# andimarafioti/faster-qwen3-tts

Hardware: NVIDIA H100
Metric: xRealTime (RTF) Qwen3-TTS-1.7B streaming chunk_size=8 (p50 TTFA in config) (higher is better)
Workload: dtype bf16

## Files before the change

### faster-qwen3-tts_b200/csrc/fq3_decode.cuh

```cuda
#pragma once
#include <cuda_bf16.h>
#include <cuda_runtime.h>
#include <stdint.h>

#include <type_traits>

#include "../../include/fq3_engine.h"

namespace fq3 {

constexpr int NCW = 8;
constexpr int NCT = NCW * 32;
constexpr int NTHREADS = NCT + 32;
constexpr int NS = 5;
constexpr int STAGE_BYTES = 32768;
constexpr int XS_FLOATS = 6144;
constexpr int HMAX = 2048;
constexpr int VMAX = 4096;
constexpr int MAXGRP = 512;
constexpr int MAXSEG = 256;
constexpr int SEQMAX = 4096;

enum Mode { MODE_FUSED = 0, MODE_TALKER_STEP = 1, MODE_PRED_RUN = 2, MODE_GEMV_TEST = 3 };

// ... 13 lines not shown
  float temperature, top_p, penalty;
};

struct StackDev {
  int H, I, L, nH, nKV, V, qd, kd, rep;
  float eps;
  int seg_base;
  int seg_head;
  const void *ln_in, *ln_post, *qnorm, *knorm, *ln_f;
  int S;
  const float *cos, *sin;
  int npos;
};

constexpr int KV_PAGE = 64;
__host__ __device__ __forceinline__ size_t kv_half_bytes(int L, int nKV, size_t esz) {
  return (size_t)L * nKV * KV_PAGE * 128 * esz;
}
__host__ __device__ __forceinline__ uint8_t* kv_row(void* pool, int L, int nKV, size_t esz, const int* pages, int which,
                                                    int layer, int g, int t) {
  const int page = pages[t / KV_PAGE];
  const size_t half = kv_half_bytes(L, nKV, esz);
  return reinterpret_cast<uint8_t*>(pool) + (size_t)page * 2 * half + (size_t)which * half +
         ((size_t)(layer * nKV + g) * KV_PAGE + t % KV_PAGE) * 128 * esz;
}

enum StateWord { ST_TOKEN = 0, ST_STEP = 1, ST_GEN = 2, ST_FIN = 3, ST_EMIT = 4, ST_WORDS = 5 };

struct SlotParams {
  void* kv;
  const int* kv_pages;
  void *pkc, *pvc;
  int* state;
  float* past_hidden;
  uint32_t* seen;
  const void* trailing;
  const void* tts_pad;
  const float* uniforms;
  long long* codes_out;
  float* logprob_out;
  int prefill_len, rope_delta, n_left_pad, max_new, min_new, trailing_len;
  int text_open;
  int n_frames;
  Sampling sp_t, sp_p;
};

struct KParams {
  StackDev t, p;
  int mode, ncta, nseg, seg_mtp;
  const uint8_t* tape;
  const Grp* grps;
  const uint32_t* segtab;
  const uint32_t* cta_grp_off;
  float *X, *X1, *QKV, *ACT, *LOGITS;
  void* ATT;
  int ldX, ldQKV, ldATT, ldACT;
  unsigned* bar;
  const void* t_embed;
  const void* p_embeds;
  const void* mtp_b;
  const void* mtp_tab;
  int has_mtp, ncb, eos, max_seq_len;
  SlotParams req;
  int n_frames;
  const void* in_embeds;
  void* hidden_out;
  int position;
  const void* pred_input;
  const float* pred_uniforms;
  float* dbg;
  int dbg_on;
  long long dbg_stride_layer;
  int attn_split;
  float* PART;
  unsigned* attn_cnt;
  int nslots;
  const SlotParams* sl;
  float *XB, *X1B, *QKVB, *LOGB;
  void *XNB, *ATTB, *ACTB, *PINB;
  int* TOKB;
  int gt_seg, gt_K, gt_ncols, gt_rows, gt_swiglu;
  const void* gt_x;
  void* gt_out;
};

__device__ __forceinline__ uint32_t smem_u32(const void* p) { return (uint32_t)__cvta_generic_to_shared(p); }
__device__ __forceinline__ void mbar_init(uint64_t* b, uint32_t cnt) {
  asm volatile("mbarrier.init.shared::cta.b64 [%0], %1;" ::"r"(smem_u32(b)), "r"(cnt) : "memory");
}
__device__ __forceinline__ void mbar_expect_tx(uint64_t* b, uint32_t bytes) {
  asm volatile("mbarrier.arrive.expect_tx.shared::cta.b64 _, [%0], %1;" ::"r"(smem_u32(b)), "r"(bytes) : "memory");
}
__device__ __forceinline__ void mbar_arrive(uint64_t* b) {
  asm volatile("mbarrier.arrive.shared::cta.b64 _, [%0];" ::"r"(smem_u32(b)) : "memory");
}
__device__ __forceinline__ bool mbar_try_wait(uint64_t* b, uint32_t parity) {
  uint32_t ok;
  asm volatile(
      "{\n\t.reg .pred p;\n\t"
      "mbarrier.try_wait.parity.shared::cta.b64 p, [%1], %2;\n\t"
      "selp.u32 %0, 1, 0, p;\n\t}"
      : "=r"(ok)
      : "r"(smem_u32(b)), "r"(parity)
      : "memory");
  return ok != 0;
}
__device__ __forceinline__ void mbar_wait(uint64_t* b, uint32_t parity) {
  while (!mbar_try_wait(b, parity)) {
// ... 812 lines not shown
    SMEM().ibc[3] = -1;
    SMEM().ibc[0] = 0x7fffffff;
  }
  csync();
  float woff = 0.f, total = 0.f;
  for (int w = 0; w < NCW; ++w) {
    if (w == c.warp) woff = total;
    total += SMEM().red[w];
  }
  incl += woff;
  const float target = a.u * total;
  float excl = __shfl_up_sync(0xffffffffu, incl, 1);
  if (c.lane == 0) excl = woff;
  const bool hit = incl > target;
  if (hit) atomicMin(&SMEM().ibc[0], c.tid);
  csync();
  if (hit && SMEM().ibc[0] == c.tid) {
    float run = excl;
    int pick = -1;
    for (int j = 0; j < CH; ++j) {
      const int idx = c.tid * CH + j;
      if (idx >= V) break;
      run += lg[idx];
      if (run > target && lg[idx] > 0.f) { pick = idx; break; }
    }
    SMEM().ibc[3] = pick;
  }
  csync();
  int tok = SMEM().ibc[3];
  if (tok < 0) {
    int best = -1;
    for (int v = c.tid; v < V; v += NCT)
      if (lg[v] > 0.f) best = v > best ? v : best;
#pragma unroll
    for (int o = 16; o; o >>= 1) best = max(best, __shfl_xor_sync(0xffffffffu, best, o));
    if (c.lane == 0) SMEM().hist[c.warp] = best;
    csync();
    tok = SMEM().hist[0];
    for (int w = 1; w < NCW; ++w) tok = max(tok, SMEM().hist[w]);
    if (tok < 0) tok = 0;
  }
  if (a.lp && c.tid == 0) *a.lp = (lraw[tok] - mx) - logf(sm);
  csync();
  return tok;
}

__device__ __forceinline__ void mma_bf16(float* d, const uint4& a, uint32_t b0, uint32_t b1) {
  asm volatile(
      "mma.sync.aligned.m16n8k16.row.col.f32.bf16.bf16.f32 {%0,%1,%2,%3}, {%4,%5,%6,%7}, {%8,%9}, {%0,%1,%2,%3};"
      : "+f"(d[0]), "+f"(d[1]), "+f"(d[2]), "+f"(d[3])
      : "r"(a.x), "r"(a.y), "r"(a.z), "r"(a.w), "r"(b0), "r"(b1));
}

template <int NT, class Pre, class Epi>
__device__ __forceinline__ void gemv_mma(Ctx& c, int seg, int K, Pre pre, Epi epi) {
  const __nv_bfloat16* xh = reinterpret_cast<const __nv_bfloat16*>(SMEM().xs);
  float* red = SMEM().xs + XS_FLOATS / 2;
  const uint32_t st = SMEM().seg[seg];
  const int gbeg = (int)(st >> 8), gn = (int)(st & 255u);
  const int gq = c.lane >> 2, t = c.lane & 3;
  for (int gi = 0; gi < gn; ++gi) {
    const Grp g = SMEM().grp[gbeg + gi];
    const int n_mt = g.rows & 0xff, kind = g.rows >> 8, G = g.m;
    int tok, koff;
    bool bvalid;
    if (kind == 1) { tok = gq >> 1; koff = (gq & 1) * (K >> 1); bvalid = gq < 2 * NT; }
    else { tok = gq; koff = 0; bvalid = gq < NT; }
    const __nv_bfloat16* xb = xh + (bvalid ? tok * K + koff : 0) + 16 * t;
    float aux[4] = {0.f, 0.f, 0.f, 0.f};
    if (c.warp < n_mt) {
      if (kind == 0) {
        const int rA = g.row0 + c.warp * 16 + gq;
        if (2 * t < NT) { aux[0] = pre(rA, 2 * t); aux[2] = pre(rA + 8, 2 * t); }
        if (2 * t + 1 < NT) { aux[1] = pre(rA, 2 * t + 1); aux[3] = pre(rA + 8, 2 * t + 1); }
      } else if (kind == 1) {
        if (t < NT) aux[0] = pre(g.row0 + gq, t);
      }
    }
    float acc[2][4];
#pragma unroll
    for (int a = 0; a < 2; ++a)
#pragma unroll
      for (int r = 0; r < 4; ++r) acc[a][r] = 0.f;
    for (int tl = 0; tl < g.ntiles; ++tl) {
      const int stage = (int)(c.tile_ctr % NS);
      const uint32_t par = (c.tile_ctr / NS) & 1u;
      mbar_wait(&SMEM().full[stage], par);
      const uint8_t* tile = SMEM().ring[stage];
      for (int qq = c.warp; qq < G; qq += NCW) {
        const int kg = tl * G + qq;
        uint4 blo = make_uint4(0, 0, 0, 0), bhi = make_uint4(0, 0, 0, 0);
        if (bvalid) {
          blo = *reinterpret_cast<const uint4*>(xb + 64 * kg);
          bhi = *reinterpret_cast<const uint4*>(xb + 64 * kg + 8);
        }
#pragma unroll
        for (int mt = 0; mt < 2; ++mt) {
          if (mt < n_mt) {
            const uint4* A = reinterpret_cast<const uint4*>(tile + ((size_t)(mt * G + qq) * 4) * 512) + c.lane;
            const uint4 a0 = A[0], a1 = A[32], a2 = A[64], a3 = A[96];
            mma_bf16(acc[mt], a0, blo.x, blo.y);
            mma_bf16(acc[mt], a1, blo.z, blo.w);
            mma_bf16(acc[mt], a2, bhi.x, bhi.y);
            mma_bf16(acc[mt], a3, bhi.z, bhi.w);
          }
        }
      }
      __syncwarp();
      if (c.lane == 0) mbar_arrive(&SMEM().empty[stage]);
      c.tile_ctr++;
    }
#pragma unroll
    for (int mt = 0; mt < 2; ++mt)
      if (mt < n_mt)
#pragma unroll
        for (int r = 0; r < 4; ++r) red[((c.warp * 2 + mt) * 4 + r) * 32 + c.lane] = acc[mt][r];
    csync();
    if (c.warp < n_mt) {
      const int mt = c.warp;
      float cv[4];
#pragma unroll
      for (int r = 0; r < 4; ++r) {
        float sm = 0.f;
#pragma unroll
        for (int w = 0; w < NCW; ++w) sm += red[((w * 2 + mt) * 4 + r) * 32 + c.lane];
        cv[r] = sm;
      }
      if (kind == 2) {
        const int pair = g.row0 + mt * 8 + gq;
        if (2 * t < NT) epi(pair, 2 * t, cv[0], cv[2], 0.f);
        if (2 * t + 1 < NT) epi(pair, 2 * t + 1, cv[1], cv[3], 0.f);
      } else if (kind == 0) {
        const int rA = g.row0 + mt * 16 + gq;
        if (2 * t < NT) { epi(rA, 2 * t, cv[0], 0.f, aux[0]); epi(rA + 8, 2 * t, cv[2], 0.f, aux[2]); }
        if (2 * t + 1 < NT) { epi(rA, 2 * t + 1, cv[1], 0.f, aux[1]); epi(rA + 8, 2 * t + 1, cv[3], 0.f, aux[3]); }
      } else {
        if (t < NT) epi(g.row0 + gq, t, cv[0] + cv[3], 0.f, aux[0]);
      }
    }
    csync();
  }
}

template <bool BF, bool GU, class Pre, class Epi>
__device__ __forceinline__ void gemv_any(Ctx& c, int seg, int nt, int K, Pre pre, Epi epi) {
  if constexpr (BF) {
    if (nt == 1) gemv_mma<1>(c, seg, K, pre, epi);
    else gemv_mma<2>(c, seg, K, pre, epi);
  } else {
    auto epi2 = [&](int row0, const float* v0, const float* v1) {
      for (int t = 0; t < nt; ++t) {
        if constexpr (GU) {
          epi(row0 >> 1, t, v0[t], v1[t], 0.f);
        } else {
          epi(row0, t, v0[t], 0.f, pre(row0, t));
          epi(row0 + 1, t, v1[t], 0.f, pre(row0 + 1, t));
        }
      }
    };
    if (nt == 1) gemv_seg<1, false>(c, seg, SMEM().xs, K, 1, epi2);
    else gemv_seg<2, false>(c, seg, SMEM().xs, K, 2, epi2);
  }
}

template <bool BF>
__device__ __forceinline__ void xs_put(Ctx& c, int idx, float v) {
  if constexpr (BF) reinterpret_cast<__nv_bfloat16*>(SMEM().xs)[idx] = __float2bfloat16_rn(v);
  else SMEM().xs[idx] = v;
}
template <bool BF>
__device__ __forceinline__ float xs_get(Ctx& c, int idx) {
  if constexpr (BF) return __bfloat162float(reinterpret_cast<const __nv_bfloat16*>(SMEM().xs)[idx]);
  else return SMEM().xs[idx];
}

template <int N, int O>
__device__ __forceinline__ void rs_step(float* a, int lane) {
  constexpr int HH = (N + 1) / 2;
  const bool up = (lane & O) != 0;
#pragma unroll
  for (int i = 0; i < HH; ++i) {
    const float lo = a[i];
    const float hi = (i + HH < N) ? a[i + HH] : 0.f;
    const float send = up ? lo : hi, keep = up ? hi : lo;
    a[i] = keep + __shfl_xor_sync(0xffffffffu, send, O);
  }
}
__host__ __device__ constexpr int rs34_lane(int idx) {
  int l = 0, r = idx;
  if (r >= 17) { l |= 16; r -= 17; }
  if (r >= 9) { l |= 8; r -= 9; }
  if (r >= 5) { l |= 4; r -= 5; }
  if (r >= 3) { l |= 2; r -= 3; }
  if (r >= 2) { l |= 1; r -= 2; }
  return l;
}
__host__ __device__ constexpr int rs34_slot(int idx) {
  int r = idx;
  if (r >= 17) r -= 17;
  if (r >= 9) r -= 9;
  if (r >= 5) r -= 5;
  if (r >= 3) r -= 3;
  if (r >= 2) r -= 2;
  return r;
}
template <int HHI = 0, int J = 0>
__device__ __forceinline__ void rs34_gather(const float* a, int lane, float* mine) {
  if constexpr (HHI < 2) {
    constexpr int idx = HHI * 17 + J;
    const float v = __shfl_sync(0xffffffffu, a[rs34_slot(idx)], rs34_lane(idx));
    if (lane == J) mine[HHI] = v;
    if constexpr (J + 1 < 17) rs34_gather<HHI, J + 1>(a, lane, mine);
    else rs34_gather<HHI + 1, 0>(a, lane, mine);
  }
}

template <bool BF>
struct SmallKV {
  using Raw = typename std::conditional<BF, uint2, float4>::type;
  Raw k[16], v[16];
};
template <bool BF>
__device__ __forceinline__ void small_kv_preload(Ctx& c, const StackDev& S, int layer, int slot0, const void* kc,
                                                 const void* vc, SmallKV<BF>& pre) {
  using Raw = typename SmallKV<BF>::Raw;
  const size_t esz = BF ? 2 : 4;
  const int g = c.warp < S.nKV ? c.warp : 0;
  const Raw* kp = reinterpret_cast<const Raw*>(reinterpret_cast<const uint8_t*>(kc) + ((size_t)(layer * S.nKV + g) * S.S * 128) * esz) + c.lane;
  const Raw* vp = reinterpret_cast<const Raw*>(reinterpret_cast<const uint8_t*>(vc) + ((size_t)(layer * S.nKV + g) * S.S * 128) * esz) + c.lane;
  constexpr int ROW = (int)(128 * (BF ? 2 : 4) / sizeof(Raw));
  Raw k[16], v[16];
#pragma unroll
  for (int j = 0; j < 16; ++j) {
    if (j < slot0) {
      k[j] = __ldcg(kp + j * ROW);
      v[j] = __ldcg(vp + j * ROW);
    } else {
      if constexpr (BF) { k[j] = make_uint2(0, 0); v[j] = make_uint2(0, 0); }
      else { k[j] = make_float4(0, 0, 0, 0); v[j] = make_float4(0, 0, 0, 0); }
    }
  }
#pragma unroll
  for (int j = 0; j < 16; ++j) {
    pre.k[j] = k[j];
    pre.v[j] = v[j];
  }
}

template <bool BF, int NT, class Out>
__device__ void attention_small_all(Ctx& c, const StackDev& S, int layer, int slot0_, int rpos0, const float* __restrict__ qkv0,
                                    size_t qkv_tstride, void* kc, void* vc, bool append, const SmallKV<BF>* pre, Out out) {
  constexpr int NOLD = NT == 2 ? 1 : 16;
  constexpr int MAXK = NT == 2 ? 2 : 17;
  const int slot0 = NT == 2 ? 0 : slot0_;
  const float scale = 0.08838834764831845f;
  const size_t esz = BF ? 2 : 4;
  const int L4 = 4 * c.lane;
  using Raw = typename std::conditional<BF, uint2, float4>::type;
  auto unpack = [](const Raw& r, float* o) {
    if constexpr (BF) { o[0] = bf_lo(r.x); o[1] = bf_hi(r.x); o[2] = bf_lo(r.y); o[3] = bf_hi(r.y); }
    else { o[0] = r.x; o[1] = r.y; o[2] = r.z; o[3] = r.w; }
  };
  auto zero_raw = [](Raw& r) {
    if constexpr (BF) r = make_uint2(0, 0);
    else r = make_float4(0, 0, 0, 0);
  };
  for (int g = c.warp; g < S.nKV; g += NCW) {
    uint8_t* kb = reinterpret_cast<uint8_t*>(kc) + ((size_t)(layer * S.nKV + g) * S.S * 128) * esz;
    uint8_t* vb = reinterpret_cast<uint8_t*>(vc) + ((size_t)(layer * S.nKV + g) * S.S * 128) * esz;
    Raw kraw[NOLD];
#pragma unroll
    for (int j = 0; j < NOLD; ++j) {
      if (pre && NT == 1 && g == c.warp) kraw[j] = pre->k[j];
      else if (j < slot0) kraw[j] = __ldcg(reinterpret_cast<const Raw*>(kb + (size_t)j * 128 * esz) + c.lane);
      else zero_raw(kraw[j]);
    }
    float4 qn4, kn4, cs4[NT], sn4[NT], kr4[NT], vr4[NT], qr4[2][NT];
    {
      float qn[4], kn[4];
#pragma unroll
      for (int i = 0; i < 4; ++i) {
        qn[i] = ldw<BF>(S.qnorm, (size_t)layer * 128 + L4 + i);
        kn[i] = ldw<BF>(S.knorm, (size_t)layer * 128 + L4 + i);
      }
      qn4 = make_float4(qn[0], qn[1], qn[2], qn[3]);
      kn4 = make_float4(kn[0], kn[1], kn[2], kn[3]);
    }
#pragma unroll
    for (int t = 0; t < NT; ++t) {
      int rp = rpos0 + t;
      rp = rp < 0 ? 0 : (rp >= S.npos ? S.npos - 1 : rp);
      cs4[t] = __ldg(reinterpret_cast<const float4*>(S.cos + (size_t)rp * 128) + c.lane);
      sn4[t] = __ldg(reinterpret_cast<const float4*>(S.sin + (size_t)rp * 128) + c.lane);
      const float* row = qkv0 + (size_t)t * qkv_tstride;
      kr4[t] = __ldcg(reinterpret_cast<const float4*>(row + S.qd + g * 128) + c.lane);
      vr4[t] = __ldcg(reinterpret_cast<const float4*>(row + S.qd + S.kd + g * 128) + c.lane);
#pragma unroll
      for (int hh = 0; hh < 2; ++hh)
        qr4[hh][t] = __ldcg(reinterpret_cast<const float4*>(row + (g * S.rep + (hh < S.rep ? hh : 0)) * 128) + c.lane);
    }
    auto norm_rope = [&](float* v, const float4& w4, const float4& c4, const float4& s4) {
      const float w[4] = {w4.x, w4.y, w4.z, w4.w}, cc[4] = {c4.x, c4.y, c4.z, c4.w}, sv[4] = {s4.x, s4.y, s4.z, s4.w};
      float ss = v[0] * v[0] + v[1] * v[1] + v[2] * v[2] + v[3] * v[3];
#pragma unroll
      for (int o = 16; o; o >>= 1) ss += __shfl_xor_sync(0xffffffffu, ss, o);
      const float r = 1.0f / sqrtf(ss / 128.0f + S.eps);
      float o4[4];
#pragma unroll
      for (int i = 0; i < 4; ++i) v[i] = rnd<BF>(w[i] * rnd<BF>(v[i] * r));
#pragma unroll
      for (int i = 0; i < 4; ++i) {
        const float other = __shfl_xor_sync(0xffffffffu, v[i], 16);
        const float rot = c.lane < 16 ? -other : other;
        o4[i] = rnd<BF>(rnd<BF>(v[i] * rnd<BF>(cc[i])) + rnd<BF>(rot * rnd<BF>(sv[i])));
      }
#pragma unroll
      for (int i = 0; i < 4; ++i) v[i] = o4[i];
    };
    float knew[NT][4], vnew[NT][4];
#pragma unroll
    for (int t = 0; t < NT; ++t) {
      knew[t][0] = kr4[t].x; knew[t][1] = kr4[t].y; knew[t][2] = kr4[t].z; knew[t][3] = kr4[t].w;
      vnew[t][0] = vr4[t].x; vnew[t][1] = vr4[t].y; vnew[t][2] = vr4[t].z; vnew[t][3] = vr4[t].w;
      norm_rope(knew[t], kn4, cs4[t], sn4[t]);
      if (append) {
#pragma unroll
        for (int i = 0; i < 4; ++i) {
          stw<BF>(kb + (size_t)(slot0 + t) * 128 * esz, L4 + i, knew[t][i]);
          stw<BF>(vb + (size_t)(slot0 + t) * 128 * esz, L4 + i, vnew[t][i]);
        }
      }
    }
    float q[2][NT][4];
#pragma unroll
    for (int hh = 0; hh < 2; ++hh)
#pragma unroll
      for (int t = 0; t < NT; ++t) {
        q[hh][t][0] = qr4[hh][t].x; q[hh][t][1] = qr4[hh][t].y; q[hh][t][2] = qr4[hh][t].z; q[hh][t][3] = qr4[hh][t].w;
        norm_rope(q[hh][t], qn4, cs4[t], sn4[t]);
      }
    float sc[2][NT][MAXK];
#pragma unroll
    for (int j = 0; j < MAXK; ++j) {
      float kf[4] = {0.f, 0.f, 0.f, 0.f};
      if (j < NOLD && j < slot0) unpack(kraw[j < NOLD ? j : 0], kf);
#pragma unroll
// ... 117 lines not shown
                                           float eps, int off, const float* wpre = nullptr) {
  constexpr int MAXE = NORM_E;
  float v[MAXE], wv[MAXE];
#pragma unroll
  for (int i = 0; i < MAXE; ++i) {
    const int k = c.tid + i * NCT;
    v[i] = 0.f;
    wv[i] = 0.f;
    if (k < H) {
      v[i] = src_smem ? src[k] : __ldcg(src + k);
      wv[i] = wpre ? wpre[i] : ldw<BF>(w, woff + k);
    }
  }
  float ss = 0.f;
#pragma unroll
  for (int i = 0; i < MAXE; ++i) ss += v[i] * v[i];
  ss = block_sum(c, ss);
  const float r = 1.0f / sqrtf(ss / (float)H + eps);
#pragma unroll
  for (int i = 0; i < MAXE; ++i) {
    const int k = c.tid + i * NCT;
    if (k < H) xs_put<BF>(c, off + k, rnd<BF>(wv[i] * rnd<BF>(v[i] * r)));
  }
  csync();
}

template <bool BF, bool TALKER>
__device__ void run_layers(Ctx& c, const StackDev& S, int nt, int slot0, int rpos0, int kv_start,
                                        bool x0_local, bool dbg) {
  constexpr bool is_talker = TALKER;
  const KParams& P = c.P;
  const bool cta0 = blockIdx.x == 0;
  void* kc = P.req.pkc;
  void* vc = P.req.pvc;
  int pi = 0;
  dbg = dbg && (P.dbg_on & 1);
  auto nopre = [](int, int) { return 0.f; };
  float wnext[NORM_E];
  for (int l = 0; l < S.L; ++l) {
    probe(c, pi);
    for (int t = 0; t < nt; ++t) {
      const float* wp = l > 0 ? wnext : nullptr;
      if (l == 0 && x0_local) norm_stage<BF>(c, SMEM().xin[t], true, S.ln_in, (size_t)l * S.H, S.H, S.eps, t * S.H, wp);
      else norm_stage<BF>(c, P.X + (size_t)t * P.ldX, false, S.ln_in, (size_t)l * S.H, S.H, S.eps, t * S.H, wp);
    }
    probe(c, pi);
    gemv_any<BF, false>(c, S.seg_base + 4 * l + 0, nt, S.H, nopre,
                        [&](int row, int t, float v, float, float) { P.QKV[(size_t)t * P.ldQKV + row] = rnd<BF>(v); });
    probe(c, pi);
    const bool small_attn = !TALKER;
    const bool kv_pre = small_attn && nt == 1;
    SmallKV<BF> skv;
    grid_arrive(c);
    if (kv_pre) small_kv_preload<BF>(c, S, l, slot0, kc, vc, skv);
    grid_wait(c);
    probe(c, pi);
    if (dbg && cta0) {
      float* d = P.dbg + (size_t)l * P.dbg_stride_layer;
      for (int t = 0; t < nt; ++t)
        for (int k = c.tid; k < S.qd + 2 * S.kd; k += NCT) d[(size_t)t * (S.qd + 2 * S.kd) + k] = __ldcg(P.QKV + (size_t)t * P.ldQKV + k);
    }
    if constexpr (!TALKER) {
      auto to_xs = [&](int t, int i, float v) { xs_put<BF>(c, t * S.qd + i, v); };
      if (nt == 1) attention_small_all<BF, 1>(c, S, l, slot0, rpos0, P.QKV, P.ldQKV, kc, vc, cta0, &skv, to_xs);
      else attention_small_all<BF, 2>(c, S, l, slot0, rpos0, P.QKV, P.ldQKV, kc, vc, cta0, nullptr, to_xs);
      probe(c, pi);
      probe(c, pi);
    } else {
      const bool split = BF && is_talker && nt == 1 && P.attn_split > 0 && slot0 - kv_start >= ATTN_SPLIT_MIN;
      if (split) attention_split<BF>(c, S, l, slot0, rpos0, kv_start);
      else
        for (int h = blockIdx.x; h < S.nH; h += gridDim.x)
          attention_head<BF>(c, S, l, h, P.QKV, P.req.kv, SMEM().kvtab, P.ATT, slot0, rpos0, kv_start);
      if (!split && is_talker && (int)blockIdx.x >= S.nH && slot0 - kv_start > 64) {
        const int ln = (l + 1) % S.L;
        const size_t esz = BF ? 2 : 4;
        const int lines_per_row = (int)(128 * esz / 128);
        const int nk = slot0 - kv_start + (ln == 0 ? 1 : 0);
        const long long total = (long long)S.nKV * nk * lines_per_row * 2;
        const int nidle = (int)gridDim.x - S.nH;
        for (long long i = (long long)(blockIdx.x - S.nH) * NCT + c.tid; i < total; i += (long long)nidle * NCT) {
          const int which = (int)(i & 1);
          long long r = i >> 1;
          const int ln_i = (int)(r % lines_per_row);
          r /= lines_per_row;
          const int j = (int)(r % nk);
          const int g = (int)(r / nk);
          const uint8_t* base = kv_row(P.req.kv, S.L, S.nKV, esz, SMEM().kvtab, which, ln, g, kv_start + j) +
                                (size_t)ln_i * 128;
          asm volatile("prefetch.global.L2::evict_last [%0];" ::"l"(base));
        }
      }
      probe(c, pi);
      grid_sync(c);
      probe(c, pi);
      {
        const uint4* att = reinterpret_cast<const uint4*>(P.ATT);
        for (int k = c.tid; k < S.qd * (BF ? 2 : 4) / 16; k += NCT) reinterpret_cast<uint4*>(SMEM().xs)[k] = __ldcg(att + k);
      }
      csync();
    }
    if (dbg && cta0) {
      float* d = P.dbg + (size_t)l * P.dbg_stride_layer + (size_t)2 * (S.qd + 2 * S.kd);
      for (int k = c.tid; k < nt * S.qd; k += NCT) d[k] = xs_get<BF>(c, k);
    }
    {
      const bool loc = (l == 0 && x0_local);
      gemv_any<BF, false>(
          c, S.seg_base + 4 * l + 1, nt, S.qd,
          [&](int row, int t) { return loc ? SMEM().xin[t][row] : __ldcg(P.X + (size_t)t * P.ldX + row); },
          [&](int row, int t, float v, float, float res) { P.X1[(size_t)t * P.ldX + row] = rnd<BF>(res + rnd<BF>(v)); });
    }
    probe(c, pi);
    float wpost[NORM_E];
    grid_arrive(c);
    norm_wload<BF>(c, S.ln_post, (size_t)l * S.H, S.H, wpost);
    grid_wait(c);
    probe(c, pi);
    for (int t = 0; t < nt; ++t)
      norm_stage<BF>(c, P.X1 + (size_t)t * P.ldX, false, S.ln_post, (size_t)l * S.H, S.H, S.eps, t * S.H, wpost);
    if (dbg && cta0) {
      float* d = P.dbg + (size_t)l * P.dbg_stride_layer + (size_t)2 * (S.qd + 2 * S.kd) + 2 * S.qd;
      for (int t = 0; t < nt; ++t)
        for (int k = c.tid; k < S.H; k += NCT) d[(size_t)t * S.H + k] = __ldcg(P.X1 + (size_t)t * P.ldX + k);
    }
    gemv_any<BF, true>(c, S.seg_base + 4 * l + 2, nt, S.H, nopre, [&](int pair, int t, float gv, float uv, float) {
      const float gte = rnd<BF>(gv), up = rnd<BF>(uv);
      const float sl = rnd<BF>(gte / (1.0f + expf(-gte)));
      P.ACT[(size_t)t * P.ldACT + pair] = rnd<BF>(sl * up);
    });
    probe(c, pi);
    grid_sync(c);
    probe(c, pi);
    for (int t = 0; t < nt; ++t) {
      constexpr int U = 12;
      for (int k0 = 0; k0 < S.I; k0 += U * NCT) {
        float v[U];
#pragma unroll
        for (int u = 0; u < U; ++u) {
          const int k = k0 + u * NCT + c.tid;
          v[u] = k < S.I ? __ldcg(P.ACT + (size_t)t * P.ldACT + k) : 0.f;
        }
#pragma unroll
        for (int u = 0; u < U; ++u) {
          const int k = k0 + u * NCT + c.tid;
          if (k < S.I) xs_put<BF>(c, t * S.I + k, v[u]);
        }
      }
    }
    csync();
    if (dbg && cta0) {
      float* d = P.dbg + (size_t)l * P.dbg_stride_layer + (size_t)2 * (S.qd + 2 * S.kd) + 2 * S.qd + 2 * S.H;
      for (int k = c.tid; k < nt * S.I; k += NCT) d[k] = xs_get<BF>(c, k);
    }
    gemv_any<BF, false>(
        c, S.seg_base + 4 * l + 3, nt, S.I, [&](int row, int t) { return __ldcg(P.X1 + (size_t)t * P.ldX + row); },
        [&](int row, int t, float v, float, float res) { P.X[(size_t)t * P.ldX + row] = rnd<BF>(res + rnd<BF>(v)); });
    probe(c, pi);
    grid_arrive(c);
    if (l + 1 < S.L) norm_wload<BF>(c, S.ln_in, (size_t)(l + 1) * S.H, S.H, wnext);
    else norm_wload<BF>(c, S.ln_f, 0, S.H, wnext);
    grid_wait(c);
    probe(c, pi);
    if (dbg && cta0) {
      float* d = P.dbg + (size_t)l * P.dbg_stride_layer + (size_t)2 * (S.qd + 2 * S.kd) + 2 * S.qd + 2 * S.H + 2 * S.I;
      for (int t = 0; t < nt; ++t)
        for (int k = c.tid; k < S.H; k += NCT) d[(size_t)t * S.H + k] = __ldcg(P.X + (size_t)t * P.ldX + k);
    }
  }
  norm_stage<BF>(c, P.X + (size_t)(nt - 1) * P.ldX, false, S.ln_f, 0, S.H, S.eps, 0, wnext);
}

template <bool BF>
__device__ __forceinline__ void head_logits(Ctx& c, int seg, int H) {
  const KParams& P = c.P;
  gemv_any<BF, false>(c, seg, 1, H, [](int, int) { return 0.f; },
                      [&](int row, int, float v, float, float) { P.LOGITS[row] = rnd<BF>(v); });
  grid_sync(c);
}

__device__ __forceinline__ SampleArgs talker_draw(const float* logits, int V, const Sampling& sp, float u,
                                                  bool suppress_special, int eos, bool suppress_eos, float* lp) {
  SampleArgs a;
  a.logits = logits; a.V = V; a.sp = sp; a.u = u;
  a.use_penalty = true; a.sup0 = suppress_special ? (V > 1024 ? V - 1024 : 0) : V;
  a.suppress_eos = suppress_eos; a.eos = eos;
  a.lp = lp;
  return a;
}
__device__ __forceinline__ SampleArgs frame_talker_draw(const KParams& P, const SlotParams& sp, const float* logits,
                                                        const float* urow, int step, float* lp_row) {
  return talker_draw(logits, P.t.V, sp.sp_t, (sp.sp_t.do_sample && urow) ? __ldg(urow) : 0.f, true, P.eos,
                     step + 1 < sp.min_new, lp_row);
}

__device__ __forceinline__ void frame_advance(int& token, int& step, int& gen_step, int next) {
  token = next;
  ++step;
  ++gen_step;
}

__device__ __forceinline__ void put_state(int* st, int token, int step, int gen_step, int finished, int emitted) {
  st[ST_TOKEN] = token; st[ST_STEP] = step; st[ST_GEN] = gen_step; st[ST_FIN] = finished; st[ST_EMIT] = emitted;
}

template <bool BF>
__device__ void predictor_frame(Ctx& cio, const float* u15, bool dbg, float* lp_row) {
  Ctx c = cio;
  const KParams& P = c.P;
  const StackDev& S = P.p;
// ... 200 lines not shown
```

### faster-qwen3-tts_b200/csrc/fq3_engine.cu

```cuda
#include <cuda_bf16.h>
#include <cuda_runtime.h>
#include <stdarg.h>
#include <stdint.h>
#include <stdio.h>
#include <string.h>

#include <algorithm>
#include <map>
#include <string>
#include <vector>

#include "../../include/fq3_engine.h"
#include "fq3_decode.cuh"
#include "fq3_decode_batch.cuh"

using namespace fq3;

static thread_local char g_err[1024] = "";
static int fail(int code, const char* fmt, ...) {
  va_list ap;
  va_start(ap, fmt);
  vsnprintf(g_err, sizeof(g_err), fmt, ap);
  va_end(ap);
  return code;
// ... 13 lines not shown
  }
  ~DevGuard() {
    if (prev >= 0 && prev != dev) cudaSetDevice(prev);
  }
};

struct SegHost {
  int rows, K;
  uint64_t bytes;
};

struct PackGrp {
  uint64_t tape_off;
  uint32_t rowsrc_idx;
  uint16_t rows, m, ntiles, pad;
  int32_t K;
};

struct SlotHost {
  bool active = false;
  int prefill_len = 0, rope_delta = 0, n_left_pad = 0, max_new = 0, min_new = 0, trailing_len = 0;
  bool text_open = false, text_closed = false;
  int step = 0;
  const void* trailing = nullptr;
  const void* tts_pad = nullptr;
  const float* uniforms = nullptr;
  Sampling sp_t{1, 50, 0.9f, 1.0f, 1.05f}, sp_p{1, 50, 0.9f, 1.0f, 1.0f};
};

struct fq3_engine {
  fq3_config cfg;
  bool bf16;
  size_t esz;
  int ncta;
  int dev;
  int max_batch = 1;
  int max_slots = 1;
  bool loaded = false;
  std::vector<SlotHost> slots;
  size_t pkv_slot = 0;
  void* kv = nullptr;
  int* kv_tab = nullptr;
  int kv_npt = 0, kv_npages = 0;
  size_t kv_page_bytes = 0;
  std::vector<int> kv_tab_host, kv_owner, kv_nmapped;
  int* kv_stage = nullptr;
  cudaStream_t kv_stream = nullptr;
  float *XB = nullptr, *X1B = nullptr, *QKVB = nullptr, *LOGB = nullptr;
  void *XNB = nullptr, *ATTB = nullptr, *ACTB = nullptr, *PINB = nullptr;
  int* TOKB = nullptr;
  SlotParams* sl_dev = nullptr;
  SlotParams* sl_host = nullptr;
  void *p_kc = nullptr, *p_vc = nullptr;
  float *X = nullptr, *X1 = nullptr, *QKV = nullptr, *ACT = nullptr, *LOGITS = nullptr, *PART = nullptr;
  void* ATT = nullptr;
  unsigned* bar = nullptr;
  int* state = nullptr;
  int* state_host = nullptr;
  float* past_hidden = nullptr;
  uint32_t* seen = nullptr;
  float* dbg = nullptr;
  size_t dbg_floats = 0;
  long long dbg_stride = 0;
  int dbg_on = 0;
  uint8_t* tape = nullptr;
  size_t tape_bytes = 0;
  Grp* grps = nullptr;
  uint32_t* segtab = nullptr;
  uint32_t* cta_grp_off = nullptr;
  std::map<std::string, void*> tabs;
  std::vector<SegHost> segs;
  int64_t talker_step_bytes = 0, predictor_frame_bytes = 0;
  KParams kp;
  int64_t launches = 0;
  const void *pf_qkv = nullptr, *pf_o = nullptr, *pf_gu = nullptr, *pf_down = nullptr, *pf_head = nullptr;
  void* pf_buf[5] = {nullptr, nullptr, nullptr, nullptr, nullptr};
  bool pf_ready = false;
};

static size_t smem_bytes() { return sizeof(Smem); }

__global__ void pack_kernel(const PackGrp* __restrict__ pg, int npg, const void* const* __restrict__ rowsrc,
                            uint8_t* __restrict__ tape) {
  for (int b = blockIdx.x; b < npg; b += gridDim.x) {
    const PackGrp g = pg[b];
    const int rows = g.rows, m = g.m;
    const long long total = (long long)rows * m * g.ntiles * 32;
    uint4* dst = reinterpret_cast<uint4*>(tape + g.tape_off);
    for (long long q = threadIdx.x; q < total; q += blockDim.x) {
      const int lane = (int)(q & 31);
      long long rem = q >> 5;
      const int j = (int)(rem % m);
      rem /= m;
      const int r = (int)(rem % rows);
      const int t = (int)(rem / rows);
      const int kb = t * m + j;
      const uint8_t* src = reinterpret_cast<const uint8_t*>(rowsrc[g.rowsrc_idx + r]);
      dst[q] = *reinterpret_cast<const uint4*>(src + ((size_t)kb * 128 + lane * 4) * 4);
    }
  }
}

__global__ void pack_mma_kernel(const PackGrp* __restrict__ pg, int npg, const void* const* __restrict__ rowsrc,
                                uint8_t* __restrict__ tape) {
  for (int b = blockIdx.x; b < npg; b += gridDim.x) {
    const int n_mt = pg[b].rows & 0xff, kind = pg[b].rows >> 8, G = pg[b].m, ntiles = pg[b].ntiles, K = pg[b].K;
    const uint32_t rowsrc_idx = pg[b].rowsrc_idx;
    const int total = ntiles * n_mt * G * 128;
// ... 147 lines not shown
static int engine_alloc(fq3_engine* e, const cudaDeviceProp& prop) {
  const fq3_config* cfg = &e->cfg;
  if (e->bf16) {
    CK(cudaFuncSetAttribute(fq3_decode_kernel<true>, cudaFuncAttributeMaxDynamicSharedMemorySize, (int)smem_bytes()));
    CK(cudaFuncSetAttribute(fq3_decode_batch_kernel<true>, cudaFuncAttributeMaxDynamicSharedMemorySize, (int)smem_bytes()));
    CK(cudaFuncSetAttribute(sample_kernel<true>, cudaFuncAttributeMaxDynamicSharedMemorySize, (int)smem_bytes()));
  } else {
    CK(cudaFuncSetAttribute(fq3_decode_kernel<false>, cudaFuncAttributeMaxDynamicSharedMemorySize, (int)smem_bytes()));
    CK(cudaFuncSetAttribute(fq3_decode_batch_kernel<false>, cudaFuncAttributeMaxDynamicSharedMemorySize, (int)smem_bytes()));
    CK(cudaFuncSetAttribute(sample_kernel<false>, cudaFuncAttributeMaxDynamicSharedMemorySize, (int)smem_bytes()));
  }
  int occ = 0;
  if (e->bf16) CK(cudaOccupancyMaxActiveBlocksPerMultiprocessor(&occ, fq3_decode_kernel<true>, NTHREADS, smem_bytes()));
  else CK(cudaOccupancyMaxActiveBlocksPerMultiprocessor(&occ, fq3_decode_kernel<false>, NTHREADS, smem_bytes()));
  if (occ < 1) return fail(FQ3_ERR_INVALID, "decode kernel does not fit on an SM (smem %zu)", smem_bytes());

  const fq3_stack_config &T = cfg->talker, &Pc = cfg->predictor;
  const int MS = e->max_slots;
  e->slots.assign(MS, SlotHost());
  const size_t pkv = pkv_bytes(*cfg, e->esz);
  e->pkv_slot = pkv;
  e->kv_npt = pages_per_seq(*cfg);
  e->kv_npages = cfg->kv_pages > 0 ? cfg->kv_pages : MS * e->kv_npt;
  e->kv_page_bytes = page_bytes(*cfg, e->esz);
  e->kv_tab_host.assign((size_t)MS * e->kv_npt, -1);
  e->kv_owner.assign(e->kv_npages, -1);
  e->kv_nmapped.assign(MS, 0);
  if (cfg->kv_pages == 0)
    for (int sl = 0; sl < MS; ++sl) {
      for (int i = 0; i < e->kv_npt; ++i) {
        e->kv_tab_host[(size_t)sl * e->kv_npt + i] = sl * e->kv_npt + i;
        e->kv_owner[sl * e->kv_npt + i] = sl;
      }
      e->kv_nmapped[sl] = e->kv_npt;
    }
  std::vector<std::pair<void*, size_t>> zero;
  auto zalloc = [&](void** p, size_t bytes) -> cudaError_t {
    cudaError_t r = cudaMalloc(p, bytes);
    if (r == cudaSuccess) zero.push_back({*p, bytes});
    return r;
  };
  CK(zalloc(&e->kv, e->kv_page_bytes * e->kv_npages));
  CK(cudaMalloc(&e->kv_tab, e->kv_tab_host.size() * sizeof(int)));
  CK(cudaMallocHost(&e->kv_stage, e->kv_npt * sizeof(int)));
  CK(cudaStreamCreateWithFlags(&e->kv_stream, cudaStreamNonBlocking));
  CK(zalloc(&e->p_kc, pkv * MS)); CK(zalloc(&e->p_vc, pkv * MS));
  const int ldX = std::max(T.hidden_size, Pc.hidden_size);
  const int ldQKV = std::max((T.num_attention_heads + 2 * T.num_key_value_heads) * 128,
                             (Pc.num_attention_heads + 2 * Pc.num_key_value_heads) * 128);
  const int ldATT = std::max(T.num_attention_heads, Pc.num_attention_heads) * 128;
  const int ldACT = std::max(T.intermediate_size, Pc.intermediate_size);
  CK(cudaMalloc(&e->X, 2 * ldX * sizeof(float))); CK(cudaMalloc(&e->X1, 2 * ldX * sizeof(float)));
  CK(cudaMalloc(&e->QKV, 2 * ldQKV * sizeof(float))); CK(cudaMalloc(&e->ATT, ldATT * e->esz));
  CK(cudaMalloc(&e->ACT, 2 * ldACT * sizeof(float))); CK(cudaMalloc(&e->LOGITS, VMAX * sizeof(float)));
  CK(zalloc((void**)&e->bar, 32768));
  CK(cudaMalloc(&e->PART, (size_t)T.num_attention_heads * 16 * PART_STRIDE * sizeof(float)));
  CK(zalloc((void**)&e->state, STATE_BYTES * MS));
  CK(cudaMallocHost(&e->state_host, STATE_BYTES * e->max_batch));
  CK(zalloc((void**)&e->past_hidden, (size_t)MS * HMAX * sizeof(float)));
  CK(zalloc((void**)&e->seen, (size_t)MS * (VMAX / 8)));
  if (e->max_batch > 1) {
    CK(zalloc((void**)&e->XB, (size_t)MAXCOL * ldX * sizeof(float)));
    CK(zalloc((void**)&e->X1B, (size_t)MAXCOL * ldX * sizeof(float)));
    CK(zalloc((void**)&e->QKVB, (size_t)MAXCOL * ldQKV * sizeof(float)));
    CK(zalloc((void**)&e->LOGB, (size_t)MAXB * VMAX * sizeof(float)));
    CK(zalloc(&e->XNB, (size_t)MAXCOL * ldX * e->esz));
    CK(zalloc(&e->ATTB, (size_t)MAXCOL * ldATT * e->esz));
    CK(zalloc(&e->ACTB, (size_t)MAXCOL * ldACT * e->esz));
    CK(zalloc(&e->PINB, (size_t)MAXCOL * HMAX * e->esz));
    CK(zalloc((void**)&e->TOKB, MAXB * sizeof(int)));
    CK(cudaMalloc(&e->sl_dev, MAXB * sizeof(SlotParams)));
    CK(cudaMallocHost(&e->sl_host, MAXB * sizeof(SlotParams)));
  }
  {
    const long long rec_t = 2LL * (T.num_attention_heads + 2 * T.num_key_value_heads) * 128 + 2LL * T.num_attention_heads * 128 + 4LL * T.hidden_size + 2LL * T.intermediate_size;
    const long long rec_p = 2LL * (Pc.num_attention_heads + 2 * Pc.num_key_value_heads) * 128 + 2LL * Pc.num_attention_heads * 128 + 4LL * Pc.hidden_size + 2LL * Pc.intermediate_size;
    e->dbg_stride = std::max(rec_t, rec_p);
    e->dbg_floats = (size_t)e->dbg_stride * std::max(T.num_hidden_layers, Pc.num_hidden_layers);
    CK(zalloc((void**)&e->dbg, e->dbg_floats * sizeof(float)));
  }
  for (auto& z : zero) CK(cudaMemset(z.first, 0, z.second));
  CK(cudaMemcpy(e->kv_tab, e->kv_tab_host.data(), e->kv_tab_host.size() * sizeof(int), cudaMemcpyHostToDevice));
  KParams& k = e->kp;
  memset(&k, 0, sizeof(k));
  auto fill = [&](StackDev& s, const fq3_stack_config& c, int S) {
    s.H = c.hidden_size; s.I = c.intermediate_size; s.L = c.num_hidden_layers;
    s.nH = c.num_attention_heads; s.nKV = c.num_key_value_heads; s.V = c.vocab_size;
    s.qd = s.nH * 128; s.kd = s.nKV * 128; s.rep = s.nH / s.nKV; s.eps = c.rms_norm_eps;
    s.S = S;
  };
  fill(k.t, T, cfg->max_seq_len);
  fill(k.p, Pc, 32);
  k.ncta = e->ncta;
  k.X = e->X; k.X1 = e->X1; k.QKV = e->QKV; k.ATT = e->ATT; k.ACT = e->ACT; k.LOGITS = e->LOGITS;
  k.ldX = ldX; k.ldQKV = ldQKV; k.ldATT = ldATT; k.ldACT = ldACT;
  k.bar = e->bar;
  k.XB = e->XB; k.X1B = e->X1B; k.QKVB = e->QKVB; k.LOGB = e->LOGB;
  k.XNB = e->XNB; k.ATTB = e->ATTB; k.ACTB = e->ACTB; k.PINB = e->PINB; k.TOKB = e->TOKB;
  k.nslots = 0; k.sl = e->sl_dev;
  k.has_mtp = cfg->has_mtp_projection; k.ncb = cfg->num_code_groups - 1; k.eos = cfg->codec_eos_token_id;
  k.max_seq_len = cfg->max_seq_len;
  k.dbg = e->dbg; k.dbg_stride_layer = e->dbg_stride;
  {
    int Sx = e->bf16 ? std::min(e->ncta / std::max(T.num_attention_heads, 1), 16) : 0;
    if (Sx < 2 || (cfg->max_seq_len + Sx - 1) / Sx > 4 * KVT_KEYS) Sx = 0;
    if (const char* v = getenv("FQ3_ATTN_SPLIT")) Sx = std::min(Sx, std::max(atoi(v), 0)) < 2 ? 0 : std::min(Sx, atoi(v));
    k.attn_split = Sx;
// ... 804 lines not shown
```

Before: 17.49.

## Read MLP down-proj activations directly from global bf16 buffer with prefetch

The MLP activation buffer becomes bf16, stored via stw. The down-projection GEMV now reads its B operand straight from global memory with __ldcg, prefetching the next tile's operands in registers, instead of first staging the whole activation vector into shared memory behind a block sync. The qnorm/knorm and RoPE cos/sin loads are also moved into the KV preload phase so they overlap the grid barrier wait. The aim is to cut the staging copy and csync on every layer's critical path, at the cost of more register pressure and L2 reads repeated per CTA.

```diff
diff --git a/faster-qwen3-tts_b200/csrc/fq3_decode.cuh b/faster-qwen3-tts_b200/csrc/fq3_decode.cuh
--- a/faster-qwen3-tts_b200/csrc/fq3_decode.cuh
+++ b/faster-qwen3-tts_b200/csrc/fq3_decode.cuh
@@ -89,8 +89,9 @@
   const Grp* grps;
   const uint32_t* segtab;
   const uint32_t* cta_grp_off;
-  float *X, *X1, *QKV, *ACT, *LOGITS;
+  float *X, *X1, *QKV, *LOGITS;
   void* ATT;
+  void* ACT;
   int ldX, ldQKV, ldATT, ldACT;
   unsigned* bar;
   const void* t_embed;
@@ -1009,9 +1010,8 @@
       : "r"(a.x), "r"(a.y), "r"(a.z), "r"(a.w), "r"(b0), "r"(b1));
 }
 
-template <int NT, class Pre, class Epi>
-__device__ __forceinline__ void gemv_mma(Ctx& c, int seg, int K, Pre pre, Epi epi) {
-  const __nv_bfloat16* xh = reinterpret_cast<const __nv_bfloat16*>(SMEM().xs);
+template <int NT, bool XG, class Pre, class Epi>
+__device__ __forceinline__ void gemv_mma(Ctx& c, int seg, int K, const __nv_bfloat16* x, int ldx, Pre pre, Epi epi) {
   float* red = SMEM().xs + XS_FLOATS / 2;
   const uint32_t st = SMEM().seg[seg];
   const int gbeg = (int)(st >> 8), gn = (int)(st & 255u);
@@ -1023,7 +1023,20 @@
     bool bvalid;
     if (kind == 1) { tok = gq >> 1; koff = (gq & 1) * (K >> 1); bvalid = gq < 2 * NT; }
     else { tok = gq; koff = 0; bvalid = gq < NT; }
-    const __nv_bfloat16* xb = xh + (bvalid ? tok * K + koff : 0) + 16 * t;
+    const __nv_bfloat16* xb = x + (bvalid ? tok * ldx + koff : 0) + 16 * t;
+    uint4 bn[2][2];
+    auto fetch_b = [&](int tl) {
+#pragma unroll
+      for (int i = 0; i < 2; ++i) {
+        const int qq = c.warp + NCW * i, kg = tl * G + qq;
+        bn[i][0] = make_uint4(0, 0, 0, 0); bn[i][1] = make_uint4(0, 0, 0, 0);
+        if (bvalid && qq < G) {
+          bn[i][0] = __ldcg(reinterpret_cast<const uint4*>(xb + 64 * kg));
+          bn[i][1] = __ldcg(reinterpret_cast<const uint4*>(xb + 64 * kg + 8));
+        }
+      }
+    };
+    if constexpr (XG) fetch_b(0);
     float aux[4] = {0.f, 0.f, 0.f, 0.f};
     if (c.warp < n_mt) {
       if (kind == 0) {
@@ -1040,14 +1053,26 @@
 #pragma unroll
       for (int r = 0; r < 4; ++r) acc[a][r] = 0.f;
     for (int tl = 0; tl < g.ntiles; ++tl) {
+      uint4 bc[2][2];
+      if constexpr (XG) {
+#pragma unroll
+        for (int i = 0; i < 2; ++i) { bc[i][0] = bn[i][0]; bc[i][1] = bn[i][1]; }
+        if (tl + 1 < g.ntiles) fetch_b(tl + 1);
+      }
       const int stage = (int)(c.tile_ctr % NS);
       const uint32_t par = (c.tile_ctr / NS) & 1u;
       mbar_wait(&SMEM().full[stage], par);
       const uint8_t* tile = SMEM().ring[stage];
-      for (int qq = c.warp; qq < G; qq += NCW) {
+#pragma unroll
+      for (int i = 0; i < 2; ++i) {
+        const int qq = c.warp + NCW * i;
+        if (qq >= G) break;
         const int kg = tl * G + qq;
         uint4 blo = make_uint4(0, 0, 0, 0), bhi = make_uint4(0, 0, 0, 0);
-        if (bvalid) {
+        if constexpr (XG) {
+          blo = bc[i][0];
+          bhi = bc[i][1];
+        } else if (bvalid) {
           blo = *reinterpret_cast<const uint4*>(xb + 64 * kg);
           bhi = *reinterpret_cast<const uint4*>(xb + 64 * kg + 8);
         }
@@ -1099,11 +1124,14 @@
   }
 }
 
-template <bool BF, bool GU, class Pre, class Epi>
-__device__ __forceinline__ void gemv_any(Ctx& c, int seg, int nt, int K, Pre pre, Epi epi) {
+template <bool BF, bool GU, bool XG = false, class Pre, class Epi>
+__device__ __forceinline__ void gemv_any(Ctx& c, int seg, int nt, int K, Pre pre, Epi epi, const void* xg = nullptr,
+                                         int ldx = 0) {
   if constexpr (BF) {
-    if (nt == 1) gemv_mma<1>(c, seg, K, pre, epi);
-    else gemv_mma<2>(c, seg, K, pre, epi);
+    const __nv_bfloat16* x = XG ? reinterpret_cast<const __nv_bfloat16*>(xg) : reinterpret_cast<const __nv_bfloat16*>(SMEM().xs);
+    const int ld = XG ? ldx : K;
+    if (nt == 1) gemv_mma<1, XG>(c, seg, K, x, ld, pre, epi);
+    else gemv_mma<2, XG>(c, seg, K, x, ld, pre, epi);
   } else {
     auto epi2 = [&](int row0, const float* v0, const float* v1) {
       for (int t = 0; t < nt; ++t) {
@@ -1115,8 +1143,10 @@
         }
       }
     };
-    if (nt == 1) gemv_seg<1, false>(c, seg, SMEM().xs, K, 1, epi2);
-    else gemv_seg<2, false>(c, seg, SMEM().xs, K, 2, epi2);
+    const float* x = XG ? reinterpret_cast<const float*>(xg) : SMEM().xs;
+    const int ld = XG ? ldx : K;
+    if (nt == 1) gemv_seg<1, XG>(c, seg, x, ld, 1, epi2);
+    else gemv_seg<2, XG>(c, seg, x, ld, 2, epi2);
   }
 }
 
@@ -1176,10 +1206,27 @@
 struct SmallKV {
   using Raw = typename std::conditional<BF, uint2, float4>::type;
   Raw k[16], v[16];
+  float4 qn, kn, cs, sn;
 };
 template <bool BF>
-__device__ __forceinline__ void small_kv_preload(Ctx& c, const StackDev& S, int layer, int slot0, const void* kc,
-                                                 const void* vc, SmallKV<BF>& pre) {
+__device__ __forceinline__ void small_norm_rope_load(Ctx& c, const StackDev& S, int layer, int rp, float4& qn4,
+                                                     float4& kn4, float4& cs4, float4& sn4) {
+  const int L4 = 4 * c.lane;
+  float qn[4], kn[4];
+#pragma unroll
+  for (int i = 0; i < 4; ++i) {
+    qn[i] = ldw<BF>(S.qnorm, (size_t)layer * 128 + L4 + i);
+    kn[i] = ldw<BF>(S.knorm, (size_t)layer * 128 + L4 + i);
+  }
+  qn4 = make_float4(qn[0], qn[1], qn[2], qn[3]);
+  kn4 = make_float4(kn[0], kn[1], kn[2], kn[3]);
+  rp = rp < 0 ? 0 : (rp >= S.npos ? S.npos - 1 : rp);
+  cs4 = __ldg(reinterpret_cast<const float4*>(S.cos + (size_t)rp * 128) + c.lane);
+  sn4 = __ldg(reinterpret_cast<const float4*>(S.sin + (size_t)rp * 128) + c.lane);
+}
+template <bool BF>
+__device__ __forceinline__ void small_kv_preload(Ctx& c, const StackDev& S, int layer, int slot0, int rpos,
+                                                 const void* kc, const void* vc, SmallKV<BF>& pre) {
   using Raw = typename SmallKV<BF>::Raw;
   const size_t esz = BF ? 2 : 4;
   const int g = c.warp < S.nKV ? c.warp : 0;
@@ -1197,11 +1244,14 @@
       else { k[j] = make_float4(0, 0, 0, 0); v[j] = make_float4(0, 0, 0, 0); }
     }
   }
+  float4 qn, kn, cs, sn;
+  if constexpr (BF) small_norm_rope_load<BF>(c, S, layer, rpos, qn, kn, cs, sn);
 #pragma unroll
   for (int j = 0; j < 16; ++j) {
     pre.k[j] = k[j];
     pre.v[j] = v[j];
   }
+  if constexpr (BF) { pre.qn = qn; pre.kn = kn; pre.cs = cs; pre.sn = sn; }
 }
 
 template <bool BF, int NT, class Out>
@@ -1233,22 +1283,14 @@
       else zero_raw(kraw[j]);
     }
     float4 qn4, kn4, cs4[NT], sn4[NT], kr4[NT], vr4[NT], qr4[2][NT];
-    {
-      float qn[4], kn[4];
-#pragma unroll
-      for (int i = 0; i < 4; ++i) {
-        qn[i] = ldw<BF>(S.qnorm, (size_t)layer * 128 + L4 + i);
-        kn[i] = ldw<BF>(S.knorm, (size_t)layer * 128 + L4 + i);
-      }
-      qn4 = make_float4(qn[0], qn[1], qn[2], qn[3]);
-      kn4 = make_float4(kn[0], kn[1], kn[2], kn[3]);
+    if (BF && pre && NT == 1) {
+      qn4 = pre->qn; kn4 = pre->kn; cs4[0] = pre->cs; sn4[0] = pre->sn;
+    } else {
+#pragma unroll
+      for (int t = 0; t < NT; ++t) small_norm_rope_load<BF>(c, S, layer, rpos0 + t, qn4, kn4, cs4[t], sn4[t]);
     }
 #pragma unroll
     for (int t = 0; t < NT; ++t) {
-      int rp = rpos0 + t;
-      rp = rp < 0 ? 0 : (rp >= S.npos ? S.npos - 1 : rp);
-      cs4[t] = __ldg(reinterpret_cast<const float4*>(S.cos + (size_t)rp * 128) + c.lane);
-      sn4[t] = __ldg(reinterpret_cast<const float4*>(S.sin + (size_t)rp * 128) + c.lane);
       const float* row = qkv0 + (size_t)t * qkv_tstride;
       kr4[t] = __ldcg(reinterpret_cast<const float4*>(row + S.qd + g * 128) + c.lane);
       vr4[t] = __ldcg(reinterpret_cast<const float4*>(row + S.qd + S.kd + g * 128) + c.lane);
@@ -1472,7 +1514,7 @@
     const bool kv_pre = small_attn && nt == 1;
     SmallKV<BF> skv;
     grid_arrive(c);
-    if (kv_pre) small_kv_preload<BF>(c, S, l, slot0, kc, vc, skv);
+    if (kv_pre) small_kv_preload<BF>(c, S, l, slot0, rpos0, kc, vc, skv);
     grid_wait(c);
     probe(c, pi);
     if (dbg && cta0) {
@@ -1547,35 +1589,24 @@
     gemv_any<BF, true>(c, S.seg_base + 4 * l + 2, nt, S.H, nopre, [&](int pair, int t, float gv, float uv, float) {
       const float gte = rnd<BF>(gv), up = rnd<BF>(uv);
       const float sl = rnd<BF>(gte / (1.0f + expf(-gte)));
-      P.ACT[(size_t)t * P.ldACT + pair] = rnd<BF>(sl * up);
+      stw<BF>(P.ACT, (size_t)t * P.ldACT + pair, rnd<BF>(sl * up));
     });
     probe(c, pi);
     grid_sync(c);
     probe(c, pi);
-    for (int t = 0; t < nt; ++t) {
-      constexpr int U = 12;
-      for (int k0 = 0; k0 < S.I; k0 += U * NCT) {
-        float v[U];
-#pragma unroll
-        for (int u = 0; u < U; ++u) {
-          const int k = k0 + u * NCT + c.tid;
-          v[u] = k < S.I ? __ldcg(P.ACT + (size_t)t * P.ldACT + k) : 0.f;
-        }
-#pragma unroll
-        for (int u = 0; u < U; ++u) {
-          const int k = k0 + u * NCT + c.tid;
-          if (k < S.I) xs_put<BF>(c, t * S.I + k, v[u]);
-        }
-      }
-    }
-    csync();
     if (dbg && cta0) {
       float* d = P.dbg + (size_t)l * P.dbg_stride_layer + (size_t)2 * (S.qd + 2 * S.kd) + 2 * S.qd + 2 * S.H;
-      for (int k = c.tid; k < nt * S.I; k += NCT) d[k] = xs_get<BF>(c, k);
-    }
-    gemv_any<BF, false>(
+      for (int t = 0; t < nt; ++t)
+        for (int k = c.tid; k < S.I; k += NCT) {
+          const size_t i = (size_t)t * P.ldACT + k;
+          if constexpr (BF) d[(size_t)t * S.I + k] = __bfloat162float(__ldcg(reinterpret_cast<const __nv_bfloat16*>(P.ACT) + i));
+          else d[(size_t)t * S.I + k] = __ldcg(reinterpret_cast<const float*>(P.ACT) + i);
+        }
+    }
+    gemv_any<BF, false, true>(
         c, S.seg_base + 4 * l + 3, nt, S.I, [&](int row, int t) { return __ldcg(P.X1 + (size_t)t * P.ldX + row); },
-        [&](int row, int t, float v, float, float res) { P.X[(size_t)t * P.ldX + row] = rnd<BF>(res + rnd<BF>(v)); });
+        [&](int row, int t, float v, float, float res) { P.X[(size_t)t * P.ldX + row] = rnd<BF>(res + rnd<BF>(v)); },
+        P.ACT, P.ldACT);
     probe(c, pi);
     grid_arrive(c);
     if (l + 1 < S.L) norm_wload<BF>(c, S.ln_in, (size_t)(l + 1) * S.H, S.H, wnext);
diff --git a/faster-qwen3-tts_b200/csrc/fq3_engine.cu b/faster-qwen3-tts_b200/csrc/fq3_engine.cu
--- a/faster-qwen3-tts_b200/csrc/fq3_engine.cu
+++ b/faster-qwen3-tts_b200/csrc/fq3_engine.cu
@@ -89,8 +89,8 @@
   SlotParams* sl_dev = nullptr;
   SlotParams* sl_host = nullptr;
   void *p_kc = nullptr, *p_vc = nullptr;
-  float *X = nullptr, *X1 = nullptr, *QKV = nullptr, *ACT = nullptr, *LOGITS = nullptr, *PART = nullptr;
-  void* ATT = nullptr;
+  float *X = nullptr, *X1 = nullptr, *QKV = nullptr, *LOGITS = nullptr, *PART = nullptr;
+  void *ATT = nullptr, *ACT = nullptr;
   unsigned* bar = nullptr;
   int* state = nullptr;
   int* state_host = nullptr;
@@ -344,7 +344,7 @@
   const int ldACT = std::max(T.intermediate_size, Pc.intermediate_size);
   CK(cudaMalloc(&e->X, 2 * ldX * sizeof(float))); CK(cudaMalloc(&e->X1, 2 * ldX * sizeof(float)));
   CK(cudaMalloc(&e->QKV, 2 * ldQKV * sizeof(float))); CK(cudaMalloc(&e->ATT, ldATT * e->esz));
-  CK(cudaMalloc(&e->ACT, 2 * ldACT * sizeof(float))); CK(cudaMalloc(&e->LOGITS, VMAX * sizeof(float)));
+  CK(cudaMalloc(&e->ACT, 2 * ldACT * e->esz)); CK(cudaMalloc(&e->LOGITS, VMAX * sizeof(float)));
   CK(zalloc((void**)&e->bar, 32768));
   CK(cudaMalloc(&e->PART, (size_t)T.num_attention_heads * 16 * PART_STRIDE * sizeof(float)));
   CK(zalloc((void**)&e->state, STATE_BYTES * MS));
```

New measurement: 18.43 (median of 6 runs). 1.05x the previous value.
